# jianfenglihg/Unsupervised_depth_OpticalFlow_egomotion

Hardware: AMD Instinct MI355X
Metric: frame-pairs/sec (832x256, geom mode) (higher is better)
Workload: dtype f32; 1 GPU; train_step: mode=geom, 832x256, batch=4/GPU, num_scales=3, fwd+bwd+Adam; global_batch=4, parallelism=dp1, hw_queues=4, stream_priorities=auto

## Files before the change

include/dfe_hip.h:

```cpp
#ifndef DFE_HIP_H
#define DFE_HIP_H

#ifdef __cplusplus
extern "C" {
#endif

#define DFE_OK 0
#define DFE_ERR_NULL (-1)
#define DFE_ERR_DIMS (-2)
#define DFE_ERR_LAUNCH (-3)
#define DFE_ERR_UNSUPPORTED (-4)
#define DFE_ERR_WORKSPACE (-5)

#define DFE_MAX_SCALES 8
#define DFE_ABI_VERSION 4

int dfe_abi_version(void);
const char* dfe_error_string(int code);

int dfe_camera_floats(void);
int dfe_prepare_cameras(const float* pose, const float* K, float* cams, int B, int ndir, int nscale,
                        const float* downscale_host, void* stream);

int dfe_pose_vec2mat_fwd(const float* vec, float* T34, float* E, int n, void* stream);
int dfe_pose_vec2mat_bwd(const float* vec, const float* gT34, const float* gE, float* gvec, int n, void* stream);

int dfe_adam_chunk(void);
int dfe_adam_step(const void* table, const int* blockmap, int nblocks, double lr, double beta1, double beta2, double eps,
                  double bias_correction1, double bias_correction2, void* stream);
int dfe_adam_step_dev(const void* table, const int* blockmap, int nblocks, double lr, double beta1, double beta2, double eps,
                      double* step_count, float* coef, void* stream);

int dfe_grad_guard_ws_bytes(int nblocks);
int dfe_grad_guard_record_bytes(void);
int dfe_grad_guard(const void* table, const int* blockmap, int nblocks, double max_norm, int skip_nonfinite, double lr, double beta1,
                   double beta2, void* ws, double* step_count, float* coef, void* record, void* stream);
int dfe_adam_tick_guarded(double lr, double beta1, double beta2, double* step_count, float* coef, const void* record, void* stream);
int dfe_adam_step_guarded(const void* table, const int* blockmap, int nblocks, double beta1, double beta2, double eps,
                          const float* coef, const void* record, void* stream);

long dfe_scatter_ws_bytes(long n);

int dfe_warp_flow_fwd(const float* x, const float* flow, float* out, int B, int C, int H, int W, int use_mask,
                      int align_corners, void* stream);
int dfe_warp_flow_bwd(const float* x, const float* flow, const float* gout, float* gflow, float* gx, void* gx_ws, int B,
                      int C, int H, int W, int use_mask, int align_corners, void* stream);

int dfe_pose_partials_floats(int B, int H, int W);
int dfe_inverse_warp2_fwd(const float* img, const float* depth, const float* ref_depth, const float* cams,
                          float* out_img, float* out_valid, float* out_pdepth, float* out_cdepth, int B, int H, int W,
                          int align_corners, void* stream);
int dfe_inverse_warp2_bwd(const float* img, const float* depth, const float* ref_depth, const float* cams,
                          const float* g_img, const float* g_pdepth, const float* g_cdepth, float* g_depth,
                          float* g_refdepth, void* g_refdepth_ws, float* g_pose, float* partials, int B, int H, int W,
                          int align_corners, void* stream);

int dfe_rigid_flow_fwd(const float* depth, const float* cams, float* out, int B, int H, int W, void* stream);
int dfe_rigid_flow_bwd(const float* depth, const float* cams, const float* gout, float* g_depth, float* g_pose,
                       float* partials, int B, int H, int W, void* stream);

int dfe_occ_masks(const float* from_l, const float* tgt, const float* from_r, float* occ_bwd, float* occ_fwd,
                  float* valid_bwd, float* valid_fwd, int B, int H, int W, void* stream);
int dfe_texture_mask(const float* img, const float* warped, const float* source, float* out, int B, int H, int W,
                     void* stream);
int dfe_dynamic_mask(const float* flow, const float* rigid, float* mask, float* score, float alpha, float beta, int B,
                     int H, int W, void* stream);

int dfe_prepare_triplets(const unsigned char* in_u8, const unsigned char* flip, float* out, int B, int H0, int W0,
// ... 33 lines not shown
                      float* g_warped, float* g_c1, float* g_c2, void* g_c2_ws, float* g_flow, int B, int C, int H,
                      int W, int align_corners, void* stream);
long dfe_pwc_level_map_bytes(int B, int H, int W);
int dfe_pwc_level_fwd_map(const float* c1, const float* c2, const float* flow, float* warped, float* x, void* map, int B, int C,
                          int H, int W, int align_corners, void* stream);
int dfe_pwc_level_bwd_map(const float* c1, const float* c2, const float* flow, const float* warped, const float* gx,
                          float* g_warped, float* g_c1, float* g_c2, void* map, float* g_flow, int B, int C, int H, int W,
                          int align_corners, void* stream);

int dfe_resize(const float* in, float* out, int planes, int inH, int inW, int outH, int outW, int mode, void* stream);
int dfe_resize_bilinear_fwd(const float* in, float* out, int planes, int inH, int inW, int outH, int outW, float mult,
                            int pre_scale, void* stream);
int dfe_resize_bilinear_bwd(const float* gout, float* gin, int planes, int inH, int inW, int outH, int outW, float mult,
                            int pre_scale, void* stream);

long dfe_glue_partials_floats(int B, int C, int H, int W);
int dfe_elu_pad_fwd(const float* x, const float* bias, float* out, int B, int C, int H, int W, int apply_elu, void* stream);
int dfe_elu_pad_bwd(const float* x, const float* bias, const float* gout, float* gx, float* gbias, float* partials,
                    int B, int C, int H, int W, int apply_elu, void* stream);
int dfe_elu_up2_cat_pad_fwd(const float* x, const float* bias, const float* skip, float* out, int B, int C1, int C2,
                            int h, int w, void* stream);
int dfe_elu_up2_cat_pad_bwd(const float* x, const float* bias, const float* gout, float* gx, float* gskip, float* gbias,
                            float* partials, int B, int C1, int C2, int h, int w, void* stream);

long dfe_disp_head_partials_floats(int B, int C, int H, int W);
int dfe_disp_head_fwd(const float* p, const float* weight, const float* bias, float* out, int B, int C, int H, int W,
                      void* stream);
int dfe_disp_head_bwd(const float* p, const float* weight, const float* out, const float* gout, float* gp, float* gweight,
                      float* gbias, float* partials, int B, int C, int H, int W, void* stream);

long dfe_flow_head_partials_floats(int B, int C, int H, int W);
int dfe_flow_head_fwd(const float* x, const float* weight, const float* bias, float* out, int B, int C, int H, int W,
                      void* stream);
int dfe_flow_head_bwd(const float* x, const float* weight, const float* gout, float* gx, float* gweight, float* gbias,
                      float* partials, int B, int C, int H, int W, void* stream);

long dfe_wgrad3x3_partials_floats(int B, int Ci, int Co, int H, int W);
int dfe_wgrad3x3_fwd(const float* p, const float* gy, float* gweight, float* partials, int B, int Ci, int Co, int H, int W,
                     void* stream);

int dfe_planeconv_supported(int B, int Ci, int Co, int H, int W);
long dfe_planeconv_ws_floats(int B, int Ci, int Co, int H, int W);
int dfe_planeconv_fwd(const float* x, const float* weight, const float* bias, float slope, float* dst1, long dst1_batch_stride,
                      float* dst2, long dst2_batch_stride, float* ws, int B, int Ci, int Co, int H, int W, void* stream);
int dfe_planeconv_dgrad(const float* gy, const float* weight, float* gx, float* ws, int B, int Ci, int Co, int H, int W,
                        void* stream);
int dfe_planeconv_wgrad(const float* gy, const float* x, float* gweight, float* ws, int B, int Ci, int Co, int H, int W,
                        void* stream);

long dfe_wino_weight_floats(int Ci, int Co);
long dfe_wino_scratch_floats(int B, int Ci, int Co, int H, int W, int P);
int dfe_wino_conv3x3(const float* x, const float* weight, float* y, long y_batch_stride, float* wbuf, long wbuf_floats, int B, int Ci,
                     int Co, int H, int W, int P, int transposed_weight, void* stream);
long dfe_wino_wgrad_floats(int B, int Ci, int Co, int H, int W, int P);
int dfe_wino_wgrad_tune(int tile, int blocks1, int blocks2, int chunk);
int dfe_wino_wgrad3x3(const float* x, long x_batch_stride, const float* gy, long gy_batch_stride, float* gweight, float* ws, int B,
                      int Ci, int Co, int H, int W, int P, void* stream);
int dfe_sconv_tune(int blocks, int rows);
long dfe_sconv_wgrad_floats(int B, int Ci, int Co, int H, int W, int K, int stride, int P);
int dfe_sconv_wgrad(const float* x, long x_batch_stride, const float* gy, long gy_batch_stride, float* gweight, float* ws, int B,
                    int Ci, int Co, int H, int W, int K, int stride, int P, void* stream);
long dfe_sconv_fwd_floats(int B, int Ci, int Co, int H, int W, int K);
int dfe_sconv_fwd(const float* x, long x_batch_stride, const float* weight, const float* bias, float slope, float* y,
                  long y_batch_stride, float* ws, int B, int Ci, int Co, int H, int W, int K, void* stream);
long dfe_sconv_dgrad_floats(int B, int Ci, int Co, int H, int W, int K);
int dfe_sconv_dgrad(const float* gy, long gy_batch_stride, const float* weight, float* gx, long gx_batch_stride, float* ws, int B,
                    int Ci, int Co, int H, int W, int K, void* stream);
int dfe_conv1x1s2_supported(int B, int Ci, int Co, int H, int W);
int dfe_conv1x1s2_fwd(const float* x, long x_batch_stride, const float* weight, float* y, long y_batch_stride, int B, int Ci, int Co,
                      int H, int W, void* stream);
long dfe_conv1x1s2_wgrad_floats(int B, int Ci, int Co, int H, int W);
int dfe_conv1x1s2_wgrad(const float* x, long x_batch_stride, const float* gy, long gy_batch_stride, float* gweight, float* ws, int B,
                        int Ci, int Co, int H, int W, void* stream);
int dfe_wino_conv3x3_dilated(const float* x, const float* weight, float* y, long y_batch_stride, float* wbuf, int B, int Ci, int Co,
                             int H, int W, int dilation, int transposed_weight, void* stream);
long dfe_wino_transform_blocks(int Ci, int Co);
int dfe_wino_transform_weights_multi(const long* table, const int* blockmap, int n_blocks, void* stream);
int dfe_wino_conv3x3_u(const float* x, const float* U, float* y, long y_batch_stride, float* part, long part_floats, int B, int Ci,
                       int Co, int H, int W, int P, int dilation, void* stream);
int dfe_wino_conv3x3_u_act(const float* x, const float* U, const float* bias, float slope, float* y, long y_batch_stride, float* y2,
                           long y2_batch_stride, float* part, long part_floats, int B, int Ci, int Co, int H, int W, int P,
                           int dilation, void* stream);

int dfe_conv1x1_small_supported(int B, int Ci, int Co, int H, int W);
int dfe_conv1x1_small_fwd(const float* x, const float* weight, const float* bias, float slope, float* y, int B, int Ci, int Co,
                          int H, int W, void* stream);
int dfe_conv1x1_small_bwd(const float* gy, const float* x, const float* weight, float* gx, float* gweight, int B, int Ci, int Co,
                          int H, int W, void* stream);

long dfe_bn_partials_floats(int G, int Bg, int C, int H, int W);
int dfe_bn_fwd(const float* x, const float* residual, const float* weight, const float* bias, float* running_mean,
               float* running_var, float* y, float* save_mean, float* save_invstd, float* partials, int G, int Bg, int C,
               int H, int W, float eps, float momentum, int relu, void* stream);
int dfe_bn_bwd(const float* x, const float* y, const float* gy, const float* weight, const float* save_mean,
               const float* save_invstd, float* gx, float* gres, float* gweight, float* gbias, float* partials,
               float* scratch_means, int G, int Bg, int C, int H, int W, int relu, void* stream);

long dfe_bias_act_partials_floats(int B, int C, int H, int W);
int dfe_bias_act_fwd(float* z, const float* bias, int B, int C, int H, int W, float slope, void* stream);
int dfe_bias_act_bwd(const float* y, const float* gy, long gy_batch_stride, float* gz, float* gbias, float* partials,
                     int B, int C, int H, int W, float slope, void* stream);

int dfe_bias_act_fwd2(const float* z, const float* bias, float* dst1, long dst1_batch_stride, float* dst2,
                      long dst2_batch_stride, int B, int C, int H, int W, float slope, void* stream);
int dfe_bias_act_bwd2(const float* y, long y_batch_stride, const float* g1, long g1_batch_stride, const float* g2,
                      long g2_batch_stride, float* gz, float* gbias, float* partials, int B, int C, int H, int W,
// ... 72 lines not shown
```

unsupervised_depth_opticalflow_egomotion_amd/csrc/ops_wino.hip:

```cpp
#include "dfe_internal.h"
#include "dfe_mfma_stage.h"
#include "dfe_device.h"
#include <hip/hip_runtime.h>
#include <algorithm>
#include <cstdlib>

namespace dfe {


struct WinoEpi { const float* bias; float slope; float* y2; long y2bs; };
__device__ __forceinline__ float wino_act(float v, float bv, float slope) { v += bv; return v > 0.0f ? v : v * slope; }

#ifndef WINO_SCHED
#define WINO_SCHED 1
#endif
constexpr int WN_CC = 16;
constexpr int WN_XP = 20;

template <bool TRANSPOSED>
__device__ __forceinline__ void wino_weight_one(const float* __restrict__ w, float* __restrict__ U, int K, int C, int Kpad, int idx) {
  const int k = idx % Kpad, c = idx / Kpad;
  float g[9];
#pragma unroll
  for (int t = 0; t < 9; ++t) {
    float v = 0.0f;
    if (k < K) v = TRANSPOSED ? w[(static_cast<long>(c) * K + k) * 9 + 8 - t] : w[(static_cast<long>(k) * C + c) * 9 + t];
    g[t] = v;
  }
  float r[4][3];
#pragma unroll
  for (int j = 0; j < 3; ++j) {
    r[0][j] = g[j];
    r[1][j] = 0.5f * ((g[j] + g[3 + j]) + g[6 + j]);
    r[2][j] = 0.5f * ((g[j] - g[3 + j]) + g[6 + j]);
    r[3][j] = g[6 + j];
  }
  float* o = U + ((static_cast<long>(k >> 5) * C + c) * 32 + (k & 31)) * 16;
#pragma unroll
  for (int i = 0; i < 4; ++i) {
    o[i * 4 + 0] = r[i][0];
    o[i * 4 + 1] = 0.5f * ((r[i][0] + r[i][1]) + r[i][2]);
    o[i * 4 + 2] = 0.5f * ((r[i][0] - r[i][1]) + r[i][2]);
    o[i * 4 + 3] = r[i][2];
  }
}

template <bool TRANSPOSED>
__global__ void __launch_bounds__(256) k_wino_weights(const float* __restrict__ w, float* __restrict__ U, int K, int C, int Kpad) {
  const int idx = blockIdx.x * 256 + threadIdx.x;
  if (idx >= Kpad * C) return;
  wino_weight_one<TRANSPOSED>(w, U, K, C, Kpad, idx);
}

__global__ void __launch_bounds__(256) k_wino_weights_multi(const long* __restrict__ table, const int* __restrict__ blockmap) {
  const long* e = table + 6L * blockmap[blockIdx.x];
  const float* w = reinterpret_cast<const float*>(e[0]);
  float* U = reinterpret_cast<float*>(e[1]);
  const int K = static_cast<int>(e[2]), C = static_cast<int>(e[3]), Kpad = (K + 31) / 32 * 32;
  const int idx = (static_cast<int>(blockIdx.x) - static_cast<int>(e[5])) * 256 + threadIdx.x;
  if (idx >= Kpad * C) return;
  if (e[4]) wino_weight_one<true>(w, U, K, C, Kpad, idx);
  else wino_weight_one<false>(w, U, K, C, Kpad, idx);
}

__global__ void __launch_bounds__(256) k_wino_sum(const float* __restrict__ part, float* __restrict__ y, long ybs, int nsp, int B, long KHW,
                                                  long HWo, WinoEpi epi) {
  const long idx = static_cast<long>(blockIdx.x) * 256 + threadIdx.x;
  if (idx >= B * KHW) return;
  float s = part[idx];
  for (int k = 1; k < nsp; ++k) s += part[static_cast<long>(k) * B * KHW + idx];
  const long b = idx / KHW, r = idx - b * KHW;
  if (epi.bias || epi.slope != 1.0f) s = wino_act(s, epi.bias ? epi.bias[r / HWo] : 0.0f, epi.slope);
  y[b * ybs + r] = s;
  if (epi.y2) epi.y2[b * epi.y2bs + r] = s;
}

template <int PP, int NW, int NH>
__global__ void __launch_bounds__(64 * NW, 2) k_wino_fwd16(const float* __restrict__ x, const float* __restrict__ U, float* __restrict__ y,
                                                       long ybs, int B, int C, int K, int H, int W, int P, int TH, int TW, int ntiles,
                                                       unsigned nkt, int dil, unsigned nsp, int cps, float* __restrict__ part, WinoEpi epi,
                                                       unsigned nitems) {
  extern __shared__ float lds[];
  const int tid = threadIdx.x, lane = tid & 63, wv = tid >> 6, n = lane & 15, kq = lane >> 4;
  for (unsigned item = blockIdx.x; item < nitems; item += gridDim.x) {
  if (item != blockIdx.x) __syncthreads();
  const unsigned lid = xcd_swizzle(item, nitems);
  const int kt = static_cast<int>(lid % nkt), sp = static_cast<int>((lid / nkt) % nsp), tb = static_cast<int>(lid / (nkt * nsp));
  const int cbeg = sp * cps, Cend = min(C, cbeg + cps);
  const int Ho = H + 2 * P - 2, Wo = W + 2 * P - 2, HW = H * W;
  const int tile = min(tb * (16 * NW) + wv * 16 + n, ntiles - 1);
  int b, ty, tx, py = 0, px = 0;
  if (PP >= 0 || dil == 1) {
    b = tile / (TH * TW);
    const int tr = tile - b * TH * TW;
    ty = tr / TW; tx = tr - ty * TW;
  } else {
    const int per_row = TW * dil, per_phase = TH * per_row, per_img = per_phase * dil;
    b = tile / per_img;
    int tr = tile - b * per_img;
    py = tr / per_phase; tr -= py * per_phase;
    ty = tr / per_row; tr -= ty * per_row;
    tx = tr / dil; px = tr - tx * dil;
  }
  const int iy0 = 2 * ty - P, ix0 = 2 * tx - P;
  constexpr bool PAIR = PP >= 0;
  constexpr bool USE_L = PP == 1 || PP == 2, USE_R = PP == 1 || PP == 0;
  unsigned off[16], inb = 0;
  bool edge_l = false, edge_r = false;
  if (PAIR) {
    const bool okL = tx >= 1, okR = 2 * tx + 3 < W, okO = 2 * tx + 1 < W;
    edge_l = USE_L && okL && n == 0;
    edge_r = USE_R && okR && (n == 15 || tx == TW - 1);
#pragma unroll
    for (int i = 0; i < 4; ++i) {
      const int yy = iy0 + i;
      const bool ok = yy >= 0 && yy < H;
      const unsigned rowb = 4u * (static_cast<unsigned>(b) * C * HW + (ok ? yy * W : 0));
      off[i] = rowb + (okO ? 8u * static_cast<unsigned>(tx) : 0u);
      off[4 + i] = rowb + (edge_l ? 8u * static_cast<unsigned>(tx - 1) : edge_r ? 8u * static_cast<unsigned>(tx + 1) : 0u);
      off[8 + i] = 0; off[12 + i] = 0;
      inb |= ok ? (1u << i) : 0u;
    }
    inb |= (okL ? 16u : 0u) | (okR ? 32u : 0u) | (okO ? 64u : 0u);
  } else {
    const int Hq = H / dil, Wq = W / dil;
#pragma unroll
    for (int i = 0; i < 4; ++i)
#pragma unroll
      for (int j = 0; j < 4; ++j) {
        const int yy = iy0 + i, xx = ix0 + j;
        const bool ok = yy >= 0 && yy < Hq && xx >= 0 && xx < Wq;
        off[i * 4 + j] = 4u * (static_cast<unsigned>(b) * C * HW + (ok ? (py + dil * yy) * W + px + dil * xx : 0));
        inb |= ok ? (1u << (i * 4 + j)) : 0u;
      }
  }
  f32x4 acc[NH][16];
#pragma unroll
  for (int h = 0; h < NH; ++h)
#pragma unroll
    for (int s = 0; s < 16; ++s) acc[h][s] = f32x4{0.0f, 0.0f, 0.0f, 0.0f};
  const float* Ut = U + static_cast<long>(kt) * C * 512;
// ... 124 lines not shown
      }
#pragma unroll
      for (int i = 0; i < 4; ++i) {
        v[i * 4 + 0] = t[i * 4] - t[i * 4 + 2];
        v[i * 4 + 1] = t[i * 4 + 1] + t[i * 4 + 2];
        v[i * 4 + 2] = t[i * 4 + 2] - t[i * 4 + 1];
        v[i * 4 + 3] = t[i * 4 + 1] - t[i * 4 + 3];
      }
      if (NH == 2 && WINO_SCHED) {
        auto mfma4 = [&](int h, int q, const f32x4& u) {
#pragma unroll
          for (int j = 0; j < 4; ++j) acc[h][4 * q + j] = __builtin_amdgcn_mfma_f32_16x16x4f32(u[j], v[4 * q + j], acc[h][4 * q + j], 0, 0, 0);
        };
        __builtin_amdgcn_sched_barrier(0);
        uc = ldU(0, 2);
        mfma4(0, 0, ua); ua = ldU(0, 3);
        mfma4(0, 1, ub); ub = ldU(1, 0);
        mfma4(0, 2, uc); uc = ldU(1, 1);
        mfma4(0, 3, ua); ua = ldU(1, 2);
        mfma4(1, 0, ub); ub = ldU(1, 3);
        mfma4(1, 1, uc);
        mfma4(1, 2, ua);
        mfma4(1, 3, ub);
#define SGB_DS(n) __builtin_amdgcn_sched_group_barrier(0x100, n, 0)
#define SGB_MFMA(n) __builtin_amdgcn_sched_group_barrier(0x008, n, 0)
        SGB_DS(1); SGB_MFMA(4); SGB_DS(1); SGB_MFMA(4); SGB_DS(1); SGB_MFMA(4); SGB_DS(1); SGB_MFMA(4); SGB_DS(1); SGB_MFMA(4); SGB_DS(1); SGB_MFMA(12);
#undef SGB_DS
#undef SGB_MFMA
        __builtin_amdgcn_sched_barrier(0);
        continue;
      }
#pragma unroll
      for (int h = 0; h < NH; ++h) {
        float u[16];
#pragma unroll
        for (int q = 0; q < 4; ++q) {
          const f32x4 w4 = *reinterpret_cast<const f32x4*>(up + h * 16 * WN_XP + 4 * q);
          u[4 * q] = w4[0]; u[4 * q + 1] = w4[1]; u[4 * q + 2] = w4[2]; u[4 * q + 3] = w4[3];
        }
#pragma unroll
        for (int s = 0; s < 16; ++s) acc[h][s] = __builtin_amdgcn_mfma_f32_16x16x4f32(u[s], v[s], acc[h][s], 0, 0, 0);
      }
    }
    if (more) {
      wstore(lds + (cur ^ 1) * SLAB);
      __syncthreads();
      cur ^= 1;
    }
  }
  if (tb * (16 * NW) + wv * 16 + n >= ntiles) continue;
  const int Hoq = (PP >= 0 || dil == 1) ? Ho : H / dil, Woq = (PP >= 0 || dil == 1) ? Wo : W / dil;
  const int oy = 2 * ty, ox = 2 * tx;
  const int sy = dil * Wo, sx = dil;
  const long kplane = static_cast<long>(Ho) * Wo;
  const long ooff = static_cast<long>(py + dil * oy) * Wo + px + dil * ox;
  float* yb = (nsp > 1 ? part + (static_cast<long>(sp) * B + b) * K * kplane : y + b * ybs) + ooff;
  const bool fused = nsp == 1 && (epi.bias != nullptr || epi.slope != 1.0f);
  float* y2b = (nsp == 1 && epi.y2) ? epi.y2 + b * epi.y2bs + ooff : nullptr;
  const bool even_w = dil == 1 && (Wo & 1) == 0;
  const bool pair_st = even_w && (reinterpret_cast<uintptr_t>(nsp > 1 ? part : y) & 7) == 0 && ((nsp > 1 ? 0 : ybs) & 1) == 0;
  const bool pair_st2 = even_w && y2b && (reinterpret_cast<uintptr_t>(epi.y2) & 7) == 0 && (epi.y2bs & 1) == 0;
#pragma unroll
  for (int h = 0; h < NH; ++h)
#pragma unroll
    for (int r = 0; r < 4; ++r) {
      const int k = kt * 32 + 16 * h + 4 * kq + r;
      if (k >= K) continue;
      float t0[4], t1[4];
#pragma unroll
      for (int s = 0; s < 4; ++s) {
        t0[s] = (acc[h][s][r] + acc[h][4 + s][r]) + acc[h][8 + s][r];
        t1[s] = (acc[h][4 + s][r] - acc[h][8 + s][r]) - acc[h][12 + s][r];
      }
      float y00 = (t0[0] + t0[1]) + t0[2], y01 = (t0[1] - t0[2]) - t0[3];
      float y10 = (t1[0] + t1[1]) + t1[2], y11 = (t1[1] - t1[2]) - t1[3];
      if (fused) {
        const float bv = epi.bias ? epi.bias[k] : 0.0f;
        y00 = wino_act(y00, bv, epi.slope); y01 = wino_act(y01, bv, epi.slope);
        y10 = wino_act(y10, bv, epi.slope); y11 = wino_act(y11, bv, epi.slope);
      }
      float* o = yb + static_cast<long>(k) * Ho * Wo;
      if (pair_st) {
        if (ox < Woq) {
          if (oy < Hoq) *reinterpret_cast<f32x2*>(o) = f32x2{y00, y01};
          if (oy + 1 < Hoq) *reinterpret_cast<f32x2*>(o + sy) = f32x2{y10, y11};
        }
      } else {
        if (oy < Hoq) {
          if (ox < Woq) o[0] = y00;
          if (ox + 1 < Woq) o[sx] = y01;
        }
        if (oy + 1 < Hoq) {
          if (ox < Woq) o[sy] = y10;
          if (ox + 1 < Woq) o[sy + sx] = y11;
        }
      }
      if (y2b) {
        float* o2 = y2b + static_cast<long>(k) * Ho * Wo;
        if (pair_st2) {
          if (ox < Woq) {
            if (oy < Hoq) *reinterpret_cast<f32x2*>(o2) = f32x2{y00, y01};
            if (oy + 1 < Hoq) *reinterpret_cast<f32x2*>(o2 + sy) = f32x2{y10, y11};
          }
        } else {
          if (oy < Hoq) {
            if (ox < Woq) o2[0] = y00;
            if (ox + 1 < Woq) o2[sx] = y01;
          }
          if (oy + 1 < Hoq) {
            if (ox < Woq) o2[sy] = y10;
            if (ox + 1 < Woq) o2[sy + sx] = y11;
          }
        }
      }
    }
  }
}

}

using namespace dfe;

static int wn_dims(int B, int Ci, int Co, int H, int W, int P) {
  if (B <= 0 || Ci <= 0 || Co <= 0 || H <= 0 || W <= 0) return DFE_ERR_DIMS;
  if (P < 0 || P > 2) return DFE_ERR_UNSUPPORTED;
  if (H + 2 * P < 3 || W + 2 * P < 3) return DFE_ERR_DIMS;
  if (static_cast<long>(B) * Ci * H * W >= (1L << 30) || static_cast<long>(Co) * H * W >= (1L << 31) || Co > 65535 * 32) return DFE_ERR_DIMS;
  return DFE_OK;
}

extern "C" long dfe_wino_weight_floats(int Ci, int Co) { return (Ci <= 0 || Co <= 0) ? 0 : static_cast<long>((Co + 31) / 32) * 32 * Ci * 16; }

extern "C" long dfe_wino_weight_floats(int Ci, int Co);

struct WinoSplit { int nsp, cps; long part_floats; };

static WinoSplit wino_split(long ntiles, int Kpad, int Ci, int B, int Co, int Ho, int Wo) {
  WinoSplit w{1, Ci, 0};
  static const bool enabled = env_int("DFE_WINO_SPLIT", 1) != 0;
  const long nblk = (ntiles + 63) / 64 * (Kpad / 32);
  if (!enabled || nblk >= 384 || Ci < 64) return w;
  int nsp = static_cast<int>((512 + nblk - 1) / nblk);
  nsp = std::min(nsp, std::min(Ci / 32, 8));
  if (nsp < 2) return w;
  w.cps = ((Ci + nsp - 1) / nsp + 7) / 8 * 8;
  w.nsp = (Ci + w.cps - 1) / w.cps;
  if (w.nsp < 2) { w.nsp = 1; w.cps = Ci; return w; }
  w.part_floats = static_cast<long>(w.nsp) * B * Co * Ho * Wo;
  return w;
}

static int wino_run(const float* x, const float* weight, float* y, long y_batch_stride, float* wbuf, float* part, long part_floats, int B,
                    int Ci, int Co, int H, int W, int P, int dil, int transposed_weight, void* stream, WinoEpi epi = WinoEpi{nullptr, 1.0f, nullptr, 0}) {
  if (!x || !y || !wbuf) return DFE_ERR_NULL;
  const int rc = wn_dims(B, Ci, Co, H, W, P);
  if (rc != DFE_OK) return rc;
  if (dil < 1 || (dil > 1 && (P != 1 || H % dil != 0 || W % dil != 0 || H / dil < 2 || W / dil < 2))) return DFE_ERR_UNSUPPORTED;
  const int Ho = dil > 1 ? H : H + 2 * P - 2, Wo = dil > 1 ? W : W + 2 * P - 2;
  if (y_batch_stride < static_cast<long>(Co) * Ho * Wo || (epi.y2 && epi.y2bs < static_cast<long>(Co) * Ho * Wo)) return DFE_ERR_DIMS;
  if ((reinterpret_cast<uintptr_t>(wbuf) & 15) != 0) return DFE_ERR_UNSUPPORTED;
  if (part && (reinterpret_cast<uintptr_t>(part) & 15) != 0) return DFE_ERR_UNSUPPORTED;
  hipStream_t st = static_cast<hipStream_t>(stream);
  const int Kpad = (Co + 31) / 32 * 32;
  const int nw = Kpad * Ci;
  if (weight) {
    if (transposed_weight) k_wino_weights<true><<<(nw + 255) / 256, 256, 0, st>>>(weight, wbuf, Co, Ci, Kpad);
    else k_wino_weights<false><<<(nw + 255) / 256, 256, 0, st>>>(weight, wbuf, Co, Ci, Kpad);
    DFE_LAUNCH_CHECK();
  }
  const int TH = (Ho / dil + 1) / 2, TW = (Wo / dil + 1) / 2;
  const long ntiles = static_cast<long>(B) * TH * TW * dil * dil;
  if (ntiles >= (1L << 31)) return DFE_ERR_DIMS;
  const size_t lds_bytes = sizeof(float) * WN_CC * 32 * WN_XP;
  {
    const unsigned nkt = Kpad / 32;
    WinoSplit sp = wino_split(ntiles, Kpad, Ci, B, Co, Ho, Wo);
    if (dil > 1 || !part || part_floats < sp.part_floats) sp = WinoSplit{1, Ci, 0};
    const int tpb = 64;
    const long nblk = (ntiles + tpb - 1) / tpb * nkt * sp.nsp;
    if (nblk >= (1L << 31)) return DFE_ERR_DIMS;
    static const bool pair_ok = env_int("DFE_WINO_PAIR", 1) != 0;
    const bool pair = pair_ok && dil == 1 && W % 2 == 0 && (reinterpret_cast<uintptr_t>(x) & 7) == 0;
    const unsigned nitems = static_cast<unsigned>(nblk);
    static const int persist = env_int("DFE_WINO_PERSIST", 0);
    const unsigned g = persist > 0 ? std::min(nitems, static_cast<unsigned>(persist)) : nitems;
    const int nt = static_cast<int>(ntiles);
    const int pp = pair ? P : -1;
#define WN_LAUNCH(PPV, NHV) k_wino_fwd16<PPV, 4, NHV><<<g, 256, lds_bytes, st>>>(x, wbuf, y, y_batch_stride, B, Ci, Co, H, W, P, TH, TW, nt, nkt, dil, static_cast<unsigned>(sp.nsp), sp.cps, part, epi, nitems)
    if (Co <= 16) {
      if (pp == 1) WN_LAUNCH(1, 1); else if (pp == 0) WN_LAUNCH(0, 1); else if (pp == 2) WN_LAUNCH(2, 1); else WN_LAUNCH(-1, 1);
    } else {
      if (pp == 1) WN_LAUNCH(1, 2); else if (pp == 0) WN_LAUNCH(0, 2); else if (pp == 2) WN_LAUNCH(2, 2); else WN_LAUNCH(-1, 2);
    }
#undef WN_LAUNCH
    DFE_LAUNCH_CHECK();
    if (sp.nsp > 1) {
      const long khw = static_cast<long>(Co) * Ho * Wo, n = B * khw;
      k_wino_sum<<<static_cast<unsigned>((n + 255) / 256), 256, 0, st>>>(part, y, y_batch_stride, sp.nsp, B, khw, static_cast<long>(Ho) * Wo, epi);
    }
  }
  DFE_LAUNCH_CHECK();
  return DFE_OK;
}

extern "C" long dfe_wino_scratch_floats(int B, int Ci, int Co, int H, int W, int P) {
  if (B <= 0 || Ci <= 0 || Co <= 0 || H <= 0 || W <= 0 || P < 0 || P > 2) return 0;
  const int Ho = H + 2 * P - 2, Wo = W + 2 * P - 2;
  if (Ho < 1 || Wo < 1) return 0;
  const int Kpad = (Co + 31) / 32 * 32;
  const long ntiles = static_cast<long>(B) * ((Ho + 1) / 2) * ((Wo + 1) / 2);
  return static_cast<long>(Kpad) * Ci * 16 + wino_split(ntiles, Kpad, Ci, B, Co, Ho, Wo).part_floats;
}

extern "C" int dfe_wino_conv3x3(const float* x, const float* weight, float* y, long y_batch_stride, float* wbuf, long wbuf_floats, int B,
                                int Ci, int Co, int H, int W, int P, int transposed_weight, void* stream) {
  if (!weight) return DFE_ERR_NULL;
  const long ufl = dfe_wino_weight_floats(Ci, Co);
  if (wbuf_floats < ufl) return DFE_ERR_WORKSPACE;
  return wino_run(x, weight, y, y_batch_stride, wbuf, wbuf ? wbuf + ufl : nullptr, wbuf_floats - ufl, B, Ci, Co, H, W, P, 1, transposed_weight, stream);
}

extern "C" int dfe_wino_conv3x3_dilated(const float* x, const float* weight, float* y, long y_batch_stride, float* wbuf, int B,
                                        int Ci, int Co, int H, int W, int dilation, int transposed_weight, void* stream) {
  if (!weight) return DFE_ERR_NULL;
  return wino_run(x, weight, y, y_batch_stride, wbuf, nullptr, 0, B, Ci, Co, H, W, 1, dilation, transposed_weight, stream);
}

extern "C" int dfe_wino_conv3x3_u(const float* x, const float* U, float* y, long y_batch_stride, float* part, long part_floats, int B, int Ci,
                                  int Co, int H, int W, int P, int dilation, void* stream) {
  return wino_run(x, nullptr, y, y_batch_stride, const_cast<float*>(U), part, part_floats, B, Ci, Co, H, W, dilation > 1 ? 1 : P, dilation, 0,
                  stream);
}

extern "C" int dfe_wino_conv3x3_u_act(const float* x, const float* U, const float* bias, float slope, float* y, long y_batch_stride, float* y2,
                                      long y2_batch_stride, float* part, long part_floats, int B, int Ci, int Co, int H, int W, int P,
                                      int dilation, void* stream) {
  return wino_run(x, nullptr, y, y_batch_stride, const_cast<float*>(U), part, part_floats, B, Ci, Co, H, W, dilation > 1 ? 1 : P, dilation, 0,
                  stream, WinoEpi{bias, slope, y2, y2_batch_stride});
}

extern "C" long dfe_wino_transform_blocks(int Ci, int Co) {
  if (Ci <= 0 || Co <= 0) return 0;
  return (static_cast<long>((Co + 31) / 32 * 32) * Ci + 255) / 256;
}

extern "C" int dfe_wino_transform_weights_multi(const long* table, const int* blockmap, int n_blocks, void* stream) {
  if (!table || !blockmap) return DFE_ERR_NULL;
  if (n_blocks <= 0) return DFE_ERR_DIMS;
  k_wino_weights_multi<<<n_blocks, 256, 0, static_cast<hipStream_t>(stream)>>>(table, blockmap);
  DFE_LAUNCH_CHECK();
  return DFE_OK;
}
```

Measured before the change: 434.6 frame-pairs/s.

## Add stream-K style balanced channel-range scheduling for Winograd forward conv

```diff
diff --git a/include/dfe_hip.h b/include/dfe_hip.h
--- a/include/dfe_hip.h
+++ b/include/dfe_hip.h
@@ -13,7 +13,7 @@
 #define DFE_ERR_WORKSPACE (-5)
 
 #define DFE_MAX_SCALES 8
-#define DFE_ABI_VERSION 4
+#define DFE_ABI_VERSION 5
 
 int dfe_abi_version(void);
 const char* dfe_error_string(int code);
@@ -153,6 +153,11 @@
 long dfe_wino_scratch_floats(int B, int Ci, int Co, int H, int W, int P);
 int dfe_wino_conv3x3(const float* x, const float* weight, float* y, long y_batch_stride, float* wbuf, long wbuf_floats, int B, int Ci,
                      int Co, int H, int W, int P, int transposed_weight, void* stream);
+int dfe_wino_plan_tune(int mode, int blocks);
+int dfe_wino_plan_query(int B, int Ci, int Co, int H, int W, int P, int* out);
+int dfe_wino_plan_segment(int B, int Ci, int Co, int H, int W, int P, int block_slot, int index, int* out);
+int dfe_wino_plan_item(int B, int Ci, int Co, int H, int W, int P, int item, int* out, int max_out);
+int dfe_wino_plan_selftest(int max_items, int max_chunks, int max_blocks);
 long dfe_wino_wgrad_floats(int B, int Ci, int Co, int H, int W, int P);
 int dfe_wino_wgrad_tune(int tile, int blocks1, int blocks2, int chunk);
 int dfe_wino_wgrad3x3(const float* x, long x_batch_stride, const float* gy, long gy_batch_stride, float* gweight, float* ws, int B,
diff --git a/unsupervised_depth_opticalflow_egomotion_amd/csrc/dfe_wino_plan.h b/unsupervised_depth_opticalflow_egomotion_amd/csrc/dfe_wino_plan.h
--- /dev/null
+++ b/unsupervised_depth_opticalflow_egomotion_amd/csrc/dfe_wino_plan.h
@@ -0,0 +1,223 @@
+#ifndef DFE_WINO_PLAN_H
+#define DFE_WINO_PLAN_H
+
+#if defined(__HIPCC__)
+#define WN_HD __host__ __device__ __forceinline__
+#else
+#define WN_HD inline
+#endif
+
+namespace dfe {
+
+constexpr int WN_SEG_FLOATS = 32 * 64 * 4;
+constexpr unsigned WN_ROUND = 512;
+
+struct WinoSeg {
+  unsigned lid;
+  int cbeg, cend;
+  int slab;
+  unsigned next;
+};
+
+WN_HD unsigned wino_cut_index(unsigned j, unsigned q) { return j - j / q; }
+
+WN_HD WinoSeg wino_range_seg(unsigned pos, unsigned end, unsigned nch, int C, unsigned L, unsigned q) {
+  WinoSeg s;
+  s.lid = pos / nch;
+  const unsigned c0 = pos - s.lid * nch;
+  const unsigned left = end - pos;
+  const unsigned c1 = (nch - c0 < left) ? nch : c0 + left;
+  s.cbeg = static_cast<int>(8 * c0);
+  s.cend = (c1 == nch) ? C : static_cast<int>(8 * c1);
+  s.next = pos + (c1 - c0);
+  const unsigned slot = pos / L;
+  if (c0 > 0) s.slab = static_cast<int>(2 * (wino_cut_index(slot, q) - 1) + 1);
+  else if (c1 < nch) s.slab = static_cast<int>(2 * (wino_cut_index(slot + 1, q) - 1));
+  else s.slab = -1;
+  return s;
+}
+
+WN_HD void wino_item_slots(unsigned lid, unsigned nch, unsigned L, unsigned* s_first, unsigned* s_last) {
+  *s_first = lid * nch / L;
+  *s_last = ((lid + 1) * nch - 1) / L;
+}
+
+WN_HD unsigned wino_item_slab(unsigned s, unsigned s_first, unsigned q) {
+  return s == s_first ? 2 * (wino_cut_index(s + 1, q) - 1) : 2 * (wino_cut_index(s, q) - 1) + 1;
+}
+
+struct WinoPlan {
+  int mode;
+  unsigned G, L, q;
+  int nsp, cps;
+  long items, nch;
+  long ncut;
+  long cut_items;
+  long segs;
+  long ws_floats;
+  double t_item, t_bal;
+};
+
+inline unsigned wino_gcd(unsigned a, unsigned b) { while (b) { const unsigned t = a % b; a = b; b = t; } return a; }
+
+inline void wino_balance(long items, long nch, long G, WinoPlan* p) {
+  const long total = items * nch;
+  if (G < 1) G = 1;
+  if (G > total) G = total;
+  const long L = (total + G - 1) / G;
+  p->L = static_cast<unsigned>(L);
+  p->G = static_cast<unsigned>((total + L - 1) / L);
+  p->q = static_cast<unsigned>(nch) / wino_gcd(p->L, static_cast<unsigned>(nch));
+  const long nb = static_cast<long>(p->G) - 1;
+  p->ncut = nb - nb / p->q;
+  long cut_items = 0, last = -1;
+  for (long j = 1; j <= nb; ++j) {
+    const long pos = j * L;
+    if (pos % nch == 0) continue;
+    if (pos / nch != last) { last = pos / nch; ++cut_items; }
+  }
+  p->cut_items = cut_items;
+  p->segs = p->ncut + cut_items;
+  p->ws_floats = 2 * p->ncut * WN_SEG_FLOATS;
+}
+
+inline void wino_uniform_split(long items, int Ci, long out_floats, WinoPlan* p) {
+  p->nsp = 1; p->cps = Ci;
+  if (items >= 384 || Ci < 64) return;
+  int nsp = static_cast<int>((512 + items - 1) / items);
+  const int cap = Ci / 32 < 8 ? Ci / 32 : 8;
+  if (nsp > cap) nsp = cap;
+  if (nsp < 2) return;
+  const int cps = ((Ci + nsp - 1) / nsp + 7) / 8 * 8;
+  nsp = (Ci + cps - 1) / cps;
+  if (nsp < 2) return;
+  p->nsp = nsp; p->cps = cps;
+  p->ws_floats = static_cast<long>(nsp) * out_floats;
+}
+
+constexpr double WN_T_CHUNK2 = 3.4;
+constexpr double WN_T_CHUNK1 = 2.4;
+constexpr double WN_T_SEG = 3.0;
+constexpr double WN_T_FIX = 10.0;
+constexpr double WN_FIX_BYTES_PER_US = 8.0e6;
+constexpr double WN_MIN_GAIN = 0.90;
+constexpr long WN_MIN_CHUNKS = 2 * WN_ROUND;
+
+inline double wino_cost_items(long blocks, long chunks) {
+  const long k = (blocks + WN_ROUND / 2 - 1) / (WN_ROUND / 2);
+  return (k / 2) * (chunks * WN_T_CHUNK2 + WN_T_SEG) + (k % 2) * (chunks * WN_T_CHUNK1 + WN_T_SEG);
+}
+
+inline double wino_cost_split(const WinoPlan& p, long out_floats) {
+  return wino_cost_items(p.items * p.nsp, p.cps / 8) + WN_T_FIX + (2.0 * p.nsp + 1.0) * out_floats * 4.0 / WN_FIX_BYTES_PER_US;
+}
+
+inline double wino_cost_balanced(const WinoPlan& p) {
+  const double per_chunk = p.G > WN_ROUND / 2 ? WN_T_CHUNK2 : WN_T_CHUNK1;
+  double t = p.L * per_chunk + WN_T_SEG * (static_cast<double>(p.L) / p.nch + 1.0);
+  if (p.ncut > 0) t += WN_T_FIX + (2.0 * p.segs + p.cut_items) * WN_SEG_FLOATS * 4.0 / WN_FIX_BYTES_PER_US;
+  return t;
+}
+
+inline WinoPlan wino_plan(int B, int Ci, int Co, int H, int W, int P, int dil, int force_mode, int force_blocks, bool allow_cut) {
+  WinoPlan w{};
+  w.mode = 1; w.nsp = 1; w.cps = Ci;
+  const int Ho = dil > 1 ? H : H + 2 * P - 2, Wo = dil > 1 ? W : W + 2 * P - 2;
+  if (B <= 0 || Ci <= 0 || Co <= 0 || Ho < 1 || Wo < 1 || dil < 1) return w;
+  const long ntiles = static_cast<long>(B) * ((Ho / dil + 1) / 2) * ((Wo / dil + 1) / 2) * dil * dil;
+  w.items = (ntiles + 63) / 64 * ((Co + 31) / 32);
+  w.nch = (Ci + 7) / 8;
+  if (!allow_cut || dil > 1 || force_mode == 1) return w;
+  const long out_floats = static_cast<long>(B) * Co * Ho * Wo;
+  const bool can_balance = w.nch >= 2 && w.items * w.nch < (1L << 30);
+  if (force_mode == 2) {
+    if (!can_balance) return w;
+    const WinoPlan whole = w;
+    wino_balance(w.items, w.nch, force_blocks > 0 ? force_blocks : WN_ROUND, &w);
+    if (w.ws_floats >= (1L << 31)) return whole;
+    w.mode = 2;
+    return w;
+  }
+  WinoPlan today = w;
+  wino_uniform_split(w.items, Ci, out_floats, &today);
+  if (today.nsp > 1) today.mode = 3;
+  if (force_mode == 3 || !can_balance || w.items * w.nch < WN_MIN_CHUNKS) return today;
+  today.t_item = today.nsp > 1 ? wino_cost_split(today, out_floats) : wino_cost_items(w.items, w.nch);
+  WinoPlan best = today;
+  const double t_best = today.t_item * WN_MIN_GAIN;
+  WinoPlan c = w;
+  wino_balance(w.items, w.nch, force_blocks > 0 ? force_blocks : WN_ROUND, &c);
+  c.t_item = today.t_item;
+  c.t_bal = wino_cost_balanced(c);
+  if (c.ncut > 0 && c.ws_floats < (1L << 31) && c.t_bal < t_best) { best = c; best.mode = 2; }
+  best.t_bal = c.t_bal;
+  return best;
+}
+
+inline int wino_plan_check(long items, long nch, long G, int C) {
+  WinoPlan p{};
+  p.items = items; p.nch = nch;
+  wino_balance(items, nch, G, &p);
+  const long total = items * nch;
+  const long Gc = G < 1 ? 1 : G > total ? total : G;
+  if (p.L != static_cast<unsigned>((total + Gc - 1) / Gc) || p.G > Gc || static_cast<long>(p.G) * p.L < total ||
+      (static_cast<long>(p.G) - 1) * p.L >= total) return 1;
+  const long nslab = p.ws_floats / WN_SEG_FLOATS;
+  long* owner = new long[total];
+  long* slab_item = new long[nslab > 0 ? nslab : 1];
+  int* slab_cbeg = new int[nslab > 0 ? nslab : 1];
+  int* slab_cend = new int[nslab > 0 ? nslab : 1];
+  for (long i = 0; i < total; ++i) owner[i] = -1;
+  for (long i = 0; i < nslab; ++i) slab_item[i] = -1;
+  int bad = 0;
+  long segs = 0;
+  for (unsigned s = 0; s < p.G && !bad; ++s) {
+    unsigned pos = s * p.L;
+    const unsigned pend = static_cast<unsigned>(pos + p.L < total ? pos + p.L : total);
+    long walked = 0;
+    while (pos < pend && !bad) {
+      const WinoSeg g = wino_range_seg(pos, pend, static_cast<unsigned>(nch), C, p.L, p.q);
+      if (g.lid >= items || g.cbeg < 0 || g.cbeg >= g.cend || g.cend > C || g.cbeg % 8 || (g.cend % 8 && g.cend != C) || g.next <= pos || g.next > pend) { bad = 2; break; }
+      for (long c = g.cbeg / 8; c < (g.cend + 7) / 8; ++c) {
+        if (owner[g.lid * nch + c] != -1) bad = 3;
+        owner[g.lid * nch + c] = s;
+        ++walked;
+      }
+      const bool partial = g.cbeg > 0 || g.cend < C;
+      if (partial != (g.slab >= 0)) bad = 4;
+      if (g.slab >= 0) {
+        if (g.slab >= nslab || slab_item[g.slab] != -1) { bad = 5; break; }
+        slab_item[g.slab] = g.lid; slab_cbeg[g.slab] = g.cbeg; slab_cend[g.slab] = g.cend;
+        ++segs;
+      }
+      pos = g.next;
+    }
+    if (!bad && walked != static_cast<long>(pend) - static_cast<long>(s) * p.L) bad = 6;
+  }
+  for (long i = 0; i < total && !bad; ++i)
+    if (owner[i] < 0) bad = 7;
+  long cut_items = 0;
+  for (long it = 0; it < items && !bad; ++it) {
+    unsigned s0, s1;
+    wino_item_slots(static_cast<unsigned>(it), static_cast<unsigned>(nch), p.L, &s0, &s1);
+    if (s0 != owner[it * nch] || s1 != owner[(it + 1) * nch - 1]) { bad = 8; break; }
+    if (s1 == s0) continue;
+    ++cut_items;
+    int at = 0;
+    for (unsigned s = s0; s <= s1; ++s) {
+      const long sl = wino_item_slab(s, s0, p.q);
+      if (sl >= nslab || slab_item[sl] != it || slab_cbeg[sl] != at) { bad = 9; break; }
+      at = slab_cend[sl];
+      slab_item[sl] = -2;
+    }
+    if (!bad && at != C) bad = 10;
+  }
+  for (long i = 0; i < nslab && !bad; ++i)
+    if (slab_item[i] >= 0) bad = 11;
+  if (!bad && (cut_items != p.cut_items || segs != p.segs || (p.ncut == 0) != (cut_items == 0))) bad = 12;
+  delete[] owner; delete[] slab_item; delete[] slab_cbeg; delete[] slab_cend;
+  return bad;
+}
+
+}
+#endif
diff --git a/unsupervised_depth_opticalflow_egomotion_amd/csrc/ops_wino.hip b/unsupervised_depth_opticalflow_egomotion_amd/csrc/ops_wino.hip
--- a/unsupervised_depth_opticalflow_egomotion_amd/csrc/ops_wino.hip
+++ b/unsupervised_depth_opticalflow_egomotion_amd/csrc/ops_wino.hip
@@ -1,6 +1,7 @@
 #include "dfe_internal.h"
 #include "dfe_mfma_stage.h"
 #include "dfe_device.h"
+#include "dfe_wino_plan.h"
 #include <hip/hip_runtime.h>
 #include <algorithm>
 #include <cstdlib>
@@ -75,18 +76,72 @@
   if (epi.y2) epi.y2[b * epi.y2bs + r] = s;
 }
 
-template <int PP, int NW, int NH>
-__global__ void __launch_bounds__(64 * NW, 2) k_wino_fwd16(const float* __restrict__ x, const float* __restrict__ U, float* __restrict__ y,
-                                                       long ybs, int B, int C, int K, int H, int W, int P, int TH, int TW, int ntiles,
-                                                       unsigned nkt, int dil, unsigned nsp, int cps, float* __restrict__ part, WinoEpi epi,
-                                                       unsigned nitems) {
+__global__ void __launch_bounds__(256) k_wino_fix(const float* __restrict__ part, float* __restrict__ y, long ybs, int K, int Ho, int Wo, int TH,
+                                                  int TW, int ntiles, unsigned nkt, unsigned nch, unsigned L, unsigned q, WinoEpi epi) {
+  const unsigned lid = blockIdx.x;
+  unsigned s0, s1;
+  wino_item_slots(lid, nch, L, &s0, &s1);
+  if (s1 == s0) return;
+  const int e = static_cast<int>(blockIdx.y) * 256 + threadIdx.x, k32 = e >> 6, t = e & 63;
+  const int kt = static_cast<int>(lid % nkt), tb = static_cast<int>(lid / nkt);
+  const int k = kt * 32 + k32, tile = tb * 64 + t;
+  if (k >= K || tile >= ntiles) return;
+  const long eo = static_cast<long>(e) * 4;
+  f32x4 s = *reinterpret_cast<const f32x4*>(part + static_cast<long>(wino_item_slab(s0, s0, q)) * WN_SEG_FLOATS + eo);
+  for (unsigned sl = s0 + 1; sl <= s1; ++sl) {
+    const f32x4 p = *reinterpret_cast<const f32x4*>(part + static_cast<long>(wino_item_slab(sl, s0, q)) * WN_SEG_FLOATS + eo);
+    s[0] += p[0]; s[1] += p[1]; s[2] += p[2]; s[3] += p[3];
+  }
+  if (epi.bias || epi.slope != 1.0f) {
+    const float bv = epi.bias ? epi.bias[k] : 0.0f;
+    s[0] = wino_act(s[0], bv, epi.slope); s[1] = wino_act(s[1], bv, epi.slope);
+    s[2] = wino_act(s[2], bv, epi.slope); s[3] = wino_act(s[3], bv, epi.slope);
+  }
+  const int b = tile / (TH * TW), tr = tile - b * TH * TW, ty = tr / TW, tx = tr - ty * TW;
+  const int oy = 2 * ty, ox = 2 * tx;
+  const long ooff = static_cast<long>(k) * Ho * Wo + static_cast<long>(oy) * Wo + ox;
+  const bool even_w = (Wo & 1) == 0;
+  auto put = [&](float* o, bool pair) {
+    if (pair) {
+      *reinterpret_cast<f32x2*>(o) = f32x2{s[0], s[1]};
+      if (oy + 1 < Ho) *reinterpret_cast<f32x2*>(o + Wo) = f32x2{s[2], s[3]};
+    } else {
+      o[0] = s[0];
+      if (ox + 1 < Wo) o[1] = s[1];
+      if (oy + 1 < Ho) {
+        o[Wo] = s[2];
+        if (ox + 1 < Wo) o[Wo + 1] = s[3];
+      }
+    }
+  };
+  put(y + b * ybs + ooff, even_w && (reinterpret_cast<uintptr_t>(y) & 7) == 0 && (ybs & 1) == 0);
+  if (epi.y2) put(epi.y2 + b * epi.y2bs + ooff, even_w && (reinterpret_cast<uintptr_t>(epi.y2) & 7) == 0 && (epi.y2bs & 1) == 0);
+}
+
+template <int PP, int NW, int NH, bool RANGED>
+__device__ __forceinline__ void wino_fwd16_body(const float* __restrict__ x, const float* __restrict__ U, float* __restrict__ y,
+                                                long ybs, int B, int C, int K, int H, int W, int P, int TH, int TW, int ntiles,
+                                                unsigned nkt, int dil, unsigned nsp, int cps, unsigned rl, unsigned rq, float* __restrict__ part,
+                                                WinoEpi epi, unsigned nitems) {
   extern __shared__ float lds[];
   const int tid = threadIdx.x, lane = tid & 63, wv = tid >> 6, n = lane & 15, kq = lane >> 4;
-  for (unsigned item = blockIdx.x; item < nitems; item += gridDim.x) {
-  if (item != blockIdx.x) __syncthreads();
-  const unsigned lid = xcd_swizzle(item, nitems);
-  const int kt = static_cast<int>(lid % nkt), sp = static_cast<int>((lid / nkt) % nsp), tb = static_cast<int>(lid / (nkt * nsp));
-  const int cbeg = sp * cps, Cend = min(C, cbeg + cps);
+  const unsigned nch = (static_cast<unsigned>(C) + 7u) >> 3;
+  const unsigned pbeg = RANGED ? xcd_swizzle(blockIdx.x, gridDim.x) * rl : blockIdx.x;
+  const unsigned pend = RANGED ? min(pbeg + rl, nitems * nch) : nitems;
+  unsigned pnext = 0;
+  for (unsigned pos = pbeg; pos < pend; pos = RANGED ? pnext : pos + gridDim.x) {
+  if (pos != pbeg) __syncthreads();
+  unsigned lid;
+  int cbeg, Cend, slab = -1, sp = 0;
+  if (RANGED) {
+    const WinoSeg sg = wino_range_seg(pos, pend, nch, C, rl, rq);
+    lid = sg.lid; cbeg = sg.cbeg; Cend = sg.cend; slab = sg.slab; pnext = sg.next;
+  } else {
+    lid = xcd_swizzle(pos, nitems);
+    sp = static_cast<int>((lid / nkt) % nsp);
+    cbeg = sp * cps; Cend = min(C, cbeg + cps);
+  }
+  const int kt = static_cast<int>(lid % nkt), tb = static_cast<int>(lid / (nkt * nsp));
   const int Ho = H + 2 * P - 2, Wo = W + 2 * P - 2, HW = H * W;
   const int tile = min(tb * (16 * NW) + wv * 16 + n, ntiles - 1);
   int b, ty, tx, py = 0, px = 0;
@@ -317,11 +372,12 @@
   const int Hoq = (PP >= 0 || dil == 1) ? Ho : H / dil, Woq = (PP >= 0 || dil == 1) ? Wo : W / dil;
   const int oy = 2 * ty, ox = 2 * tx;
   const int sy = dil * Wo, sx = dil;
+  const long ooff = static_cast<long>(py + dil * oy) * Wo + px + dil * ox;
   const long kplane = static_cast<long>(Ho) * Wo;
-  const long ooff = static_cast<long>(py + dil * oy) * Wo + px + dil * ox;
   float* yb = (nsp > 1 ? part + (static_cast<long>(sp) * B + b) * K * kplane : y + b * ybs) + ooff;
   const bool fused = nsp == 1 && (epi.bias != nullptr || epi.slope != 1.0f);
   float* y2b = (nsp == 1 && epi.y2) ? epi.y2 + b * epi.y2bs + ooff : nullptr;
+  float* pb = part + static_cast<long>(slab < 0 ? 0 : slab) * WN_SEG_FLOATS + (wv * 16 + n) * 4;
   const bool even_w = dil == 1 && (Wo & 1) == 0;
   const bool pair_st = even_w && (reinterpret_cast<uintptr_t>(nsp > 1 ? part : y) & 7) == 0 && ((nsp > 1 ? 0 : ybs) & 1) == 0;
   const bool pair_st2 = even_w && y2b && (reinterpret_cast<uintptr_t>(epi.y2) & 7) == 0 && (epi.y2bs & 1) == 0;
@@ -339,6 +395,10 @@
       }
       float y00 = (t0[0] + t0[1]) + t0[2], y01 = (t0[1] - t0[2]) - t0[3];
       float y10 = (t1[0] + t1[1]) + t1[2], y11 = (t1[1] - t1[2]) - t1[3];
+      if (RANGED && slab >= 0) {
+        *reinterpret_cast<f32x4*>(pb + (16 * h + 4 * kq + r) * 256) = f32x4{y00, y01, y10, y11};
+        continue;
+      }
       if (fused) {
         const float bv = epi.bias ? epi.bias[k] : 0.0f;
         y00 = wino_act(y00, bv, epi.slope); y01 = wino_act(y01, bv, epi.slope);
@@ -382,6 +442,22 @@
   }
 }
 
+template <int PP, int NW, int NH>
+__global__ void __launch_bounds__(64 * NW, 2) k_wino_fwd16(const float* __restrict__ x, const float* __restrict__ U, float* __restrict__ y,
+                                                       long ybs, int B, int C, int K, int H, int W, int P, int TH, int TW, int ntiles,
+                                                       unsigned nkt, int dil, unsigned nsp, int cps, float* __restrict__ part, WinoEpi epi,
+                                                       unsigned nitems) {
+  wino_fwd16_body<PP, NW, NH, false>(x, U, y, ybs, B, C, K, H, W, P, TH, TW, ntiles, nkt, dil, nsp, cps, 0u, 1u, part, epi, nitems);
+}
+
+template <int PP, int NW, int NH>
+__global__ void __launch_bounds__(64 * NW, 2) k_wino_range16(const float* __restrict__ x, const float* __restrict__ U, float* __restrict__ y,
+                                                         long ybs, int B, int C, int K, int H, int W, int P, int TH, int TW, int ntiles,
+                                                         unsigned nkt, unsigned rl, unsigned rq, float* __restrict__ part, WinoEpi epi,
+                                                         unsigned nitems) {
+  wino_fwd16_body<PP, NW, NH, true>(x, U, y, ybs, B, C, K, H, W, P, TH, TW, ntiles, nkt, 1, 1u, C, rl, rq, part, epi, nitems);
+}
+
 }
 
 using namespace dfe;
@@ -398,21 +474,77 @@
 
 extern "C" long dfe_wino_weight_floats(int Ci, int Co);
 
-struct WinoSplit { int nsp, cps; long part_floats; };
-
-static WinoSplit wino_split(long ntiles, int Kpad, int Ci, int B, int Co, int Ho, int Wo) {
-  WinoSplit w{1, Ci, 0};
+static int g_wn_tune[2] = {0, 0};
+
+static WinoPlan wino_plan_for(int B, int Ci, int Co, int H, int W, int P, int dil) {
   static const bool enabled = env_int("DFE_WINO_SPLIT", 1) != 0;
-  const long nblk = (ntiles + 63) / 64 * (Kpad / 32);
-  if (!enabled || nblk >= 384 || Ci < 64) return w;
-  int nsp = static_cast<int>((512 + nblk - 1) / nblk);
-  nsp = std::min(nsp, std::min(Ci / 32, 8));
-  if (nsp < 2) return w;
-  w.cps = ((Ci + nsp - 1) / nsp + 7) / 8 * 8;
-  w.nsp = (Ci + w.cps - 1) / w.cps;
-  if (w.nsp < 2) { w.nsp = 1; w.cps = Ci; return w; }
-  w.part_floats = static_cast<long>(w.nsp) * B * Co * Ho * Wo;
-  return w;
+  return wino_plan(B, Ci, Co, H, W, P, dil, g_wn_tune[0], g_wn_tune[1], enabled);
+}
+
+extern "C" int dfe_wino_plan_tune(int mode, int blocks) {
+  if (mode < 0 || mode > 3 || blocks < 0) return DFE_ERR_UNSUPPORTED;
+  g_wn_tune[0] = mode; g_wn_tune[1] = blocks;
+  return DFE_OK;
+}
+
+extern "C" int dfe_wino_plan_query(int B, int Ci, int Co, int H, int W, int P, int* out) {
+  if (!out) return DFE_ERR_NULL;
+  const int rc = wn_dims(B, Ci, Co, H, W, P);
+  if (rc != DFE_OK) return rc;
+  const WinoPlan p = wino_plan_for(B, Ci, Co, H, W, P, 1);
+  const bool bal = p.mode == 2, spl = p.mode == 3;
+  out[0] = p.mode;
+  out[1] = bal ? static_cast<int>(p.G) : spl ? static_cast<int>(p.items * p.nsp) : 0;
+  out[2] = bal ? static_cast<int>(p.L) : spl ? p.cps / 8 : 0;
+  out[3] = bal ? static_cast<int>(p.cut_items) : spl ? static_cast<int>(p.items) : 0;
+  out[4] = p.mode == 1 ? 0 : static_cast<int>(p.ws_floats);
+  return DFE_OK;
+}
+
+extern "C" int dfe_wino_plan_segment(int B, int Ci, int Co, int H, int W, int P, int block_slot, int index, int* out) {
+  if (!out) return DFE_ERR_NULL;
+  const int rc = wn_dims(B, Ci, Co, H, W, P);
+  if (rc != DFE_OK) return rc;
+  const WinoPlan p = wino_plan_for(B, Ci, Co, H, W, P, 1);
+  if (p.mode != 2 || block_slot < 0 || static_cast<unsigned>(block_slot) >= p.G || index < 0) return DFE_ERR_DIMS;
+  const unsigned nch = static_cast<unsigned>(p.nch), total = static_cast<unsigned>(p.items * p.nch);
+  unsigned pos = static_cast<unsigned>(block_slot) * p.L;
+  const unsigned pend = std::min(pos + p.L, total);
+  for (int i = 0; pos < pend; ++i) {
+    const WinoSeg s = wino_range_seg(pos, pend, nch, Ci, p.L, p.q);
+    if (i == index) {
+      out[0] = static_cast<int>(s.lid); out[1] = s.cbeg; out[2] = s.cend; out[3] = s.slab;
+      return 1;
+    }
+    pos = s.next;
+  }
+  return 0;
+}
+
+extern "C" int dfe_wino_plan_item(int B, int Ci, int Co, int H, int W, int P, int item, int* out, int max_out) {
+  if (!out) return DFE_ERR_NULL;
+  const int rc = wn_dims(B, Ci, Co, H, W, P);
+  if (rc != DFE_OK) return rc;
+  const WinoPlan p = wino_plan_for(B, Ci, Co, H, W, P, 1);
+  if (p.mode != 2 || item < 0 || item >= p.items) return DFE_ERR_DIMS;
+  unsigned s0, s1;
+  wino_item_slots(static_cast<unsigned>(item), static_cast<unsigned>(p.nch), p.L, &s0, &s1);
+  if (s1 == s0) return 0;
+  int n = 0;
+  for (unsigned s = s0; s <= s1; ++s, ++n)
+    if (n < max_out) out[n] = static_cast<int>(wino_item_slab(s, s0, p.q));
+  return n;
+}
+
+extern "C" int dfe_wino_plan_selftest(int max_items, int max_chunks, int max_blocks) {
+  for (int items = 1; items <= max_items; ++items)
+    for (int nch = 2; nch <= max_chunks; ++nch)
+      for (int g = 1; g <= max_blocks; ++g)
+        for (int rag = 0; rag < 8; rag += 7) {
+          const int bad = wino_plan_check(items, nch, g, 8 * nch - rag);
+          if (bad) return ((items * 100 + nch) * 100 + g) * 100 + bad;
+        }
+  return 0;
 }
 
 static int wino_run(const float* x, const float* weight, float* y, long y_batch_stride, float* wbuf, float* part, long part_floats, int B,
@@ -439,19 +571,26 @@
   const size_t lds_bytes = sizeof(float) * WN_CC * 32 * WN_XP;
   {
     const unsigned nkt = Kpad / 32;
-    WinoSplit sp = wino_split(ntiles, Kpad, Ci, B, Co, Ho, Wo);
-    if (dil > 1 || !part || part_floats < sp.part_floats) sp = WinoSplit{1, Ci, 0};
+    WinoPlan pl = wino_plan_for(B, Ci, Co, H, W, P, dil);
+    if (pl.mode != 1 && pl.ws_floats > 0 && (!part || part_floats < pl.ws_floats)) { pl.mode = 1; pl.nsp = 1; pl.cps = Ci; }
+    const bool balanced = pl.mode == 2;
+    const int nsp = pl.mode == 3 ? pl.nsp : 1, cps = pl.mode == 3 ? pl.cps : Ci;
     const int tpb = 64;
-    const long nblk = (ntiles + tpb - 1) / tpb * nkt * sp.nsp;
+    const long nblk = (ntiles + tpb - 1) / tpb * nkt * nsp;
     if (nblk >= (1L << 31)) return DFE_ERR_DIMS;
     static const bool pair_ok = env_int("DFE_WINO_PAIR", 1) != 0;
     const bool pair = pair_ok && dil == 1 && W % 2 == 0 && (reinterpret_cast<uintptr_t>(x) & 7) == 0;
     const unsigned nitems = static_cast<unsigned>(nblk);
     static const int persist = env_int("DFE_WINO_PERSIST", 0);
-    const unsigned g = persist > 0 ? std::min(nitems, static_cast<unsigned>(persist)) : nitems;
+    const unsigned g = balanced ? pl.G : persist > 0 ? std::min(nitems, static_cast<unsigned>(persist)) : nitems;
+    const unsigned rl = balanced ? pl.L : 0u, rq = balanced ? pl.q : 1u;
     const int nt = static_cast<int>(ntiles);
     const int pp = pair ? P : -1;
-#define WN_LAUNCH(PPV, NHV) k_wino_fwd16<PPV, 4, NHV><<<g, 256, lds_bytes, st>>>(x, wbuf, y, y_batch_stride, B, Ci, Co, H, W, P, TH, TW, nt, nkt, dil, static_cast<unsigned>(sp.nsp), sp.cps, part, epi, nitems)
+#define WN_LAUNCH(PPV, NHV)                                                                                                                 \
+  do {                                                                                                                                      \
+    if (balanced) k_wino_range16<PPV, 4, NHV><<<g, 256, lds_bytes, st>>>(x, wbuf, y, y_batch_stride, B, Ci, Co, H, W, P, TH, TW, nt, nkt, rl, rq, part, epi, nitems); \
+    else k_wino_fwd16<PPV, 4, NHV><<<g, 256, lds_bytes, st>>>(x, wbuf, y, y_batch_stride, B, Ci, Co, H, W, P, TH, TW, nt, nkt, dil, static_cast<unsigned>(nsp), cps, part, epi, nitems); \
+  } while (0)
     if (Co <= 16) {
       if (pp == 1) WN_LAUNCH(1, 1); else if (pp == 0) WN_LAUNCH(0, 1); else if (pp == 2) WN_LAUNCH(2, 1); else WN_LAUNCH(-1, 1);
     } else {
@@ -459,10 +598,12 @@
     }
 #undef WN_LAUNCH
     DFE_LAUNCH_CHECK();
-    if (sp.nsp > 1) {
+    if (nsp > 1) {
       const long khw = static_cast<long>(Co) * Ho * Wo, n = B * khw;
-      k_wino_sum<<<static_cast<unsigned>((n + 255) / 256), 256, 0, st>>>(part, y, y_batch_stride, sp.nsp, B, khw, static_cast<long>(Ho) * Wo, epi);
-    }
+      k_wino_sum<<<static_cast<unsigned>((n + 255) / 256), 256, 0, st>>>(part, y, y_batch_stride, nsp, B, khw, static_cast<long>(Ho) * Wo, epi);
+    }
+    if (balanced && pl.ncut > 0)
+      k_wino_fix<<<dim3(nitems, 8), 256, 0, st>>>(part, y, y_batch_stride, Co, Ho, Wo, TH, TW, nt, nkt, static_cast<unsigned>(pl.nch), pl.L, pl.q, epi);
   }
   DFE_LAUNCH_CHECK();
   return DFE_OK;
@@ -472,9 +613,8 @@
   if (B <= 0 || Ci <= 0 || Co <= 0 || H <= 0 || W <= 0 || P < 0 || P > 2) return 0;
   const int Ho = H + 2 * P - 2, Wo = W + 2 * P - 2;
   if (Ho < 1 || Wo < 1) return 0;
-  const int Kpad = (Co + 31) / 32 * 32;
-  const long ntiles = static_cast<long>(B) * ((Ho + 1) / 2) * ((Wo + 1) / 2);
-  return static_cast<long>(Kpad) * Ci * 16 + wino_split(ntiles, Kpad, Ci, B, Co, Ho, Wo).part_floats;
+  const WinoPlan pl = wino_plan_for(B, Ci, Co, H, W, P, 1);
+  return dfe_wino_weight_floats(Ci, Co) + (pl.mode != 1 ? pl.ws_floats : 0);
 }
 
 extern "C" int dfe_wino_conv3x3(const float* x, const float* weight, float* y, long y_batch_stride, float* wbuf, long wbuf_floats, int B,
```

New measurement: 434.2 frame-pairs/s. Within noise of the previous version (-0.1%).
